# szpajder/dumphfdl

Hardware: AMD Instinct MI355X
Metric: wideband I/Q Msamples/s (cf32 ingest -> decoded HFDL PDUs) at fixed channel count (higher is better)
Workload: dtype f32

## Files before the change

dumphfdl_amd/csrc/demod_core.h:

```cpp
#pragma once
#include <hip/hip_runtime.h>
#include "demod_logic.h"
#include "demod_lds.h"

namespace hfdl {

constexpr int DM_WAVES = 4, DM_THREADS = 64 * DM_WAVES;

__device__ __forceinline__ float dpp_row_shr1(float old, float src)
{
	return __int_as_float(__builtin_amdgcn_update_dpp(__float_as_int(old), __float_as_int(src), 0x111, 0xf, 0xf, false));
}
__device__ __forceinline__ float dpp_row_shl1(float old, float src)
{
	return __int_as_float(__builtin_amdgcn_update_dpp(__float_as_int(old), __float_as_int(src), 0x101, 0xf, 0xf, false));
}
__device__ __forceinline__ float dpp_row_shl2(float old, float src)
{
	return __int_as_float(__builtin_amdgcn_update_dpp(__float_as_int(old), __float_as_int(src), 0x102, 0xf, 0xf, false));
}
__device__ __forceinline__ float dpp_row_ror1(float src)
{
	return __int_as_float(__builtin_amdgcn_update_dpp(0, __float_as_int(src), 0x121, 0xf, 0xf, false));
}
// ... 95 lines not shown

__device__ __forceinline__ cf input_sample(const DemodInput &in, int g)
{
	int b = 0, start = 0;
#pragma unroll
	for (int u = 0; u < DM_MAX_BLOCKS - 1; u++) {
		const int e = in.ends[u];
		if (g >= e) { b = u + 1; start = e; }
	}
	return in.chan[(size_t)b * in.blk_stride + (size_t)(g - start)];
}

template <bool TAPS>
__device__ __forceinline__ void resample_outputs(uint32_t rs_phase, const DemodConst &T, const BlockIo &io, const cf *ring, int k0, int k1, int lane)
{
	const int k = k0 + lane;
	if (k < k1) {
		const uint64_t t = (uint64_t)rs_phase + (uint64_t)k * T.rs_step;
		const int i = (int)(t >> 24);
		const float *h = T.rs_h + ((t & 0xFFFFFFu) >> 16) * D_RS_TAPS;
		float ar = 0, ai = 0;
		for (int j = 0; j < D_RS_TAPS; j++) {
			const cf x = ring[(i - j) & DM_IN_MASK];
			ar += h[j] * x.x;
			ai += h[j] * x.y;
		}
		cf v; v.x = ar; v.y = ai;
		io.rs[k & DM_MASK] = v;
		if (TAPS) io.tap_resampled[k] = v;
	}
}


struct SymsyncRegs {
	float rate, del, tau, bf, q, qhat, v1;
	int b, decim, j;
	int valid_from;
};

__device__ __forceinline__ void symsync_load(SymsyncRegs &r, const ChanScalars &s, const ChanArrays &a, const BlockIo &io, int lane)
{
	if (lane < SS_HIST) {
		cf v; v.x = 0.f; v.y = 0.f;
		if (lane < D_SS_TAPS) v = a.ss_dmf[lane == 0 ? 0 : D_SS_TAPS - lane];
		io.mf[-1 - lane] = v;
	}
	r.rate = s.ss_rate; r.del = s.ss_del; r.tau = s.ss_tau; r.bf = s.ss_bf; r.q = s.ss_q; r.qhat = s.ss_qhat; r.v1 = s.ss_v1;
	r.b = s.ss_b; r.decim = (int)s.ss_decim; r.j = 0;
	r.valid_from = s.ss_head;
}

__device__ __forceinline__ void symsync_restart(SymsyncRegs &r, const DemodShared &sh, int k0)
{
	r.rate = 1.5f; r.del = 1.5f; r.tau = 0.f; r.bf = 0.f; r.q = 0.f; r.qhat = 0.f; r.v1 = 0.f;
	r.b = 0; r.decim = 0;
	r.j = k0 > 0 ? (int)sh.cum[(k0 - 1) & DM_MASK] : 0;
	r.valid_from = k0;
}

__device__ __forceinline__ void symsync_store(const SymsyncRegs &r, ChanScalars &s, ChanArrays &a, const BlockIo &io, int n_out, int lane)
{
	if (lane < D_SS_TAPS) a.ss_dmf[lane == 0 ? 0 : D_SS_TAPS - lane] = io.mf[((n_out - 1) & DM_MASK) - lane];
	if (lane == 0) {
		s.ss_rate = r.rate; s.ss_del = r.del; s.ss_tau = r.tau; s.ss_bf = r.bf; s.ss_q = r.q; s.ss_qhat = r.qhat; s.ss_v1 = r.v1;
		s.ss_b = r.b; s.ss_decim = (uint32_t)r.decim;
		const int vf = r.valid_from - n_out;
		s.ss_head = vf < -64 ? -64 : vf;
	}
}

template <bool MASKED>
__device__ __forceinline__ void symsync_chunk(SymsyncRegs &r, const DemodConst &T, const BlockIo &io, const DemodShared &sh, int k0, int k1, int lane)
{
	const int row = lane >> 4, t = lane & 15;
	const float *base = (const float *)(io.mf - (k0 & ~DM_MASK) - t) + (row & 1);
	int bi = r.b < 0 ? 0 : (r.b >= D_SS_NPFB ? D_SS_NPFB - 1 : r.b);
	float2 h = sh.sstab[bi * 64 + lane];
	float w_lo = base[2 * k0], w_hi = base[2 * (k0 - 16)];
	const bool out_lane = lane == 15 || lane == 31;
	float *const out_base = out_lane ? (float *)sh.outq + (lane == 31 ? 1 : 0) : sh.sink + lane;
	const int out_stride = out_lane ? 2 : 0;
	int cum_v = 0;
	for (int k = k0; k < k1; k++) {
		const float n_lo = base[2 * (k + 1)], n_hi = base[2 * (k + 1 - 16)];
		if (r.b < D_SS_NPFB) {
			float wl = w_lo, wh = w_hi;
			if (MASKED && k - (D_SS_TAPS - 1) < r.valid_from && row < 2) {
				if (k - t < r.valid_from) wl = 0.f;
				if (k - t - 16 < r.valid_from) wh = 0.f;
			}
			int produced = 0;
			do {
				const float p = row_scan_sum(h.x * wl + h.y * wh);
				if (__builtin_expect(r.j < sh.outq_cap, 1)) out_base[out_stride * (r.j & (OUTQ_RING - 1))] = div3(p);
				r.j++;
				if (r.decim == 2) {
					r.decim = 0;
					const float mx = lane_value(p, 15), my = lane_value(p, 31);
					const float dx = lane_value(p, 47), dy = lane_value(p, 63);
					float q = mx * dx + my * dy;
					q = q > 1.0f ? 1.0f : (q < -1.0f ? -1.0f : q);
					r.q = q;
					const float v0 = q - T.lf_a1 * r.v1;
					r.qhat = T.lf_b0 * v0;
					r.v1 = v0;
					r.rate += T.ss_rate_adj * r.qhat;
					r.del = r.rate + r.qhat;
				}
				r.decim++;
				r.tau += r.del;
				r.bf = r.tau * (float)D_SS_NPFB;
				r.b = (int)roundf(r.bf);
				produced++;
				if (r.b < D_SS_NPFB) h = sh.sstab[(r.b < 0 ? 0 : r.b) * 64 + lane];
			} while (r.b < D_SS_NPFB && produced < 4);
		}
		r.tau -= 1.0f;
		r.bf -= (float)D_SS_NPFB;
		r.b -= D_SS_NPFB;
		bi = r.b < 0 ? 0 : (r.b >= D_SS_NPFB ? D_SS_NPFB - 1 : r.b);
		h = sh.sstab[bi * 64 + lane];
		cum_v = (lane == k - k0) ? (r.j < 65535 ? r.j : 65535) : cum_v;
		w_lo = n_lo; w_hi = n_hi;
	}
	if (lane < k1 - k0) sh.cum[(k0 + lane) & DM_MASK] = (uint16_t)cum_v;
}


struct CarrierRegs {
	float eu, ev, ex2, ewx, ewy;
	float px, py;
#ifdef HFDL_DM_PROBE
	unsigned long long pa = 0, pb = 0, pc = 0;
#endif
};

struct LaneSlicer {
	float px, py;
	int lane;
	__device__ __forceinline__ uint32_t operator()(int arity, cf x, float *phase_error) const
	{
		uint32_t sym;
		cf xh;
		if (arity == 1) {
			sym = (x.x > 0) ? 0 : 1;
			xh.x = sym ? -1.0f : 1.0f; xh.y = 0.0f;
		} else {
			const int M = 1 << arity, base = M - 2;
			const bool mine = lane >= base && lane < base + M;
			const float d = mine ? x.x * px + x.y * py : -1.0f;
			const float best = lane_value(row_scan_max(d), 15);
			const unsigned long long hit = __builtin_amdgcn_fcmpf(d, best, 1 );
			int win = hit ? (int)__builtin_ctzll(hit) : base;
			const uint32_t lin = (uint32_t)(win - base);
			sym = lin ^ (lin >> 1);
			xh.x = lane_value(px, win); xh.y = lane_value(py, win);
		}
		if (phase_error) *phase_error = x.y * xh.x - x.x * xh.y;
		return sym;
	}
};

__device__ __forceinline__ void carrier_load(CarrierRegs &c, const ChanScalars &s, const ChanArrays &a, const DemodConst &T, int lane)
{
	c.px = lane < 16 ? T.psk_pts[2 * lane] : 0.f;
	c.py = lane < 16 ? T.psk_pts[2 * lane + 1] : 0.f;
	const int t = (lane & 15) - 1;
	const bool act = t >= 0 && lane < 32, row1 = (lane >> 4) & 1;
	int j = s.eq_head + t; if (j >= D_EQ) j -= D_EQ;
	const cf e = act ? a.eq_buf[j] : cf{0.f, 0.f};
	c.eu = row1 ? e.y : e.x;
	c.ev = row1 ? -e.x : e.y;
	c.ex2 = act ? a.eq_x2[j] : 0.f;
	const cf w = act ? a.eq_w[t] : cf{0.f, 0.f};
	c.ewx = w.x; c.ewy = w.y;
}

__device__ __forceinline__ void carrier_store(const CarrierRegs &c, ChanArrays &a, int lane)
{
	if (lane >= 1 && lane <= D_EQ) {
		cf e; e.x = c.eu; e.y = c.ev;
		a.eq_buf[lane - 1] = e; a.eq_x2[lane - 1] = c.ex2;
		cf w; w.x = c.ewx; w.y = c.ewy;
		a.eq_w[lane - 1] = w;
	}
}

template <bool TAPS>
__device__ __forceinline__ int carrier_chunk(CarrierRegs &c, ChanScalars &s, ChanArrays &a, const DemodConst &T, const BlockIo &io, const DemodShared &sh,
		int k0, int &k1, int &nsym, int lane)
{
	const int t = (lane & 15) - 1;
	const bool row1 = (lane >> 4) & 1, act = t >= 0 && lane < 32;
	int n = k1 - k0;
	const float lv_l = (lane < n) ? io.lvl[(k0 + lane) & DM_MASK] : 0.f;
	const int cum_l = (lane < n) ? (int)sh.cum[(k0 + lane) & DM_MASK] : 0x7fffffff;
	const int jbase = k0 > 0 ? (int)sh.cum[(k0 - 1) & DM_MASK] : 0;
	const cf oq_l = (jbase + lane < sh.outq_cap) ? sh.outq[(jbase + lane) & (OUTQ_RING - 1)] : cf{0.f, 0.f};
	{
#ifndef HFDL_DM_OUT_LANES
#define HFDL_DM_OUT_LANES 64
#endif
		const unsigned long long over = __ballot(lane < n && cum_l - jbase > HFDL_DM_OUT_LANES);
		if (__builtin_expect(over != 0, 0)) { n = (int)__builtin_ctzll(over); k1 = k0 + n; }
	}
	int jstop = __builtin_amdgcn_readlane(cum_l, n - 1);
	if (jstop > sh.outq_cap) jstop = sh.outq_cap;
	const uint64_t cnt0 = s.sample_cnt;
	int kdone = 0;
	int reset_at = -1;
	int staged = 0, stage_at = 0;
	auto flush_stage = [&]() {
		if (lane < staged) io.data[stage_at + lane] = sh.stage[lane];
		staged = 0;
	};
	auto catch_up = [&](int upto) {
		if (s.fr_state == FR_A1) {
			const uint32_t d = (uint32_t)(upto + 1 - kdone), c0 = s.nf_clk;
			uint32_t first = (NF_CLK_MASK - c0) & NF_CLK_MASK;
			if (first == 0) first = NF_CLK_MASK + 1;
			s.nf_clk = (uint32_t)__builtin_amdgcn_readfirstlane((int)(c0 + d));
			if (first <= d) {
				const float level = lane_value(lv_l, kdone + (int)first - 1);
				s.noise_floor = NF_KEEP * s.noise_floor + NF_TAKE * fminf(s.noise_floor, level) + NF_BIAS;
			}
		}
		kdone = upto + 1;
	};
	bool runaway = fabsf(s.dphi) > COSTAS_RUNAWAY_DPHI && s.fr_state == FR_A1;
	const int pair_sel = (lane & 1) << 2;
	auto pair_step = [&](int j) {
		const int sel = ((j - jbase) << 2) + pair_sel;
		cf oi;
		oi.x = __int_as_float(__builtin_amdgcn_ds_bpermute(sel, __float_as_int(oq_l.x)));
		oi.y = __int_as_float(__builtin_amdgcn_ds_bpermute(sel, __float_as_int(oq_l.y)));
		float ph1, ph2;
		{
			const float ph = s.phi + s.dphi;
			const float dn = ph - (float)(2.0 * M_PI), up = ph + (float)(2.0 * M_PI);
			ph1 = ph > (float)M_PI ? dn : (ph < -(float)M_PI ? up : ph);
		}
		{
			const float ph = ph1 + s.dphi;
			const float dn = ph - (float)(2.0 * M_PI), up = ph + (float)(2.0 * M_PI);
			ph2 = ph > (float)M_PI ? dn : (ph < -(float)M_PI ? up : ph);
		}
		s.phi = ph2;
#ifdef HFDL_DM_LIBM_TRIG
		float sp, cp;
		sincosf((lane & 1) ? ph2 : ph1, &sp, &cp);
#else
// ... 24 lines not shown
		const float bx = row1 ? -c.ev : c.eu, by = row1 ? c.eu : c.ev;
		const float pr = er * bx - ei * by, pi = er * by + ei * bx;
		c.ewx = c.ewx + EQ_STEP * pr / s.eq_x2sum;
		c.ewy = c.ewy + EQ_STEP * pi / s.eq_x2sum;
	};
	auto in_frame_run = [&](int &j) {
		if (!(s.symsync_out_idx & 1u) && j + 1 < jstop && s.fr_state >= FR_EQ_TRAIN && s.symbols_wanted > 1 && s.s_state == SAMPLER_SYMBOLS) {
			const bool train = s.fr_state == FR_EQ_TRAIN;
			int n_run = (jstop - j) >> 1;
			if (n_run > s.symbols_wanted - 1) n_run = s.symbols_wanted - 1;
			if ((!train || s.eq_full) && (!s.use_data || s.data_n + n_run <= MAX_DATA_SYMBOLS)) {
				if (s.use_data && staged == 0) stage_at = s.data_slot * MAX_DATA_SYMBOLS + s.data_n;
#if defined(HFDL_DM_PROBE) && HFDL_DM_PROBE >= 2
				const unsigned long long tR0 = __builtin_amdgcn_s_memtime();
#endif
				int ki = 0;
				for (int i = 0; i < n_run; i++, j += 2) {
					pair_step(j);
					const cf y = equalise();
					if (train) { train_step(y); s.T_idx++; }
					if (TAPS && lane == 0) io.tap_symbols[nsym] = y;
					nsym++;
					ki = (int)__builtin_ctzll(__ballot(cum_l > j + 1));
					const float level = lane_value(lv_l, ki);
					float perr;
					LaneSlicer{c.px, c.py, lane}(s.cur_arity, y, &perr);
					const float e = 0.5f * (fabsf(perr + COSTAS_ERR_LIMIT) - fabsf(perr - COSTAS_ERR_LIMIT));
					s.err = e;
					s.phi += COSTAS_ALPHA * e;
					s.dphi += COSTAS_BETA * e;
					if (s.use_data) sh.stage[staged++] = y;
					else if (s.training_n < T_LEN) {
						a.training[s.training_n] = y;
						s.training_n++;
					}
					s.signal_level = (s.signal_level * s.frame_symbol_cnt + level) / (s.frame_symbol_cnt + 1.0f);
					s.frame_symbol_cnt += 1.0f;
				}
				if (ki >= kdone) kdone = ki + 1;
				s.eq_count += 2u * (uint32_t)n_run;
				s.symsync_out_idx += 2u * (uint32_t)n_run;
				s.symbol_cnt += (uint64_t)n_run;
				s.symbols_wanted -= n_run;
				if (s.use_data) s.data_n += n_run;
#if defined(HFDL_DM_PROBE) && HFDL_DM_PROBE >= 2
				{
					const unsigned long long dt = HFDL_DM_PROBE == 2 ? __builtin_amdgcn_s_memtime() - tR0 : (unsigned long long)n_run;
					if (train) c.pb += dt; else c.pc += dt;
				}
#endif
			}
		}
	};
	int j = jbase;
	if (s.fr_state != FR_A1) in_frame_run(j);
	while (j < jstop) {
#ifdef HFDL_DM_PROBE
		const unsigned long long tA0 = __builtin_amdgcn_s_memtime();
		const int st0 = s.fr_state;
#endif
		int jo;
		bool on_time;
		if (!(s.symsync_out_idx & 1u) && j + 1 < jstop && !runaway) {
			pair_step(j);
			s.eq_count += 2;
			jo = j + 1; j += 2; s.symsync_out_idx += 2;
			on_time = true;
		} else {
			cf oi;
			oi.x = lane_value(oq_l.x, j - jbase); oi.y = lane_value(oq_l.y, j - jbase);
			{
				const float ph = s.phi + s.dphi;
				const float dn = ph - (float)(2.0 * M_PI), up = ph + (float)(2.0 * M_PI);
				s.phi = ph > (float)M_PI ? dn : (ph < -(float)M_PI ? up : ph);
			}
#ifdef HFDL_DM_LIBM_TRIG
			float sp, cp;
			sincosf(s.phi, &sp, &cp);
#else
			const float rev = s.phi * 0.15915494309189535f;
			const float sp = __builtin_amdgcn_sinf(rev), cp = __builtin_amdgcn_cosf(rev);
#endif
			cf r;
			r.x = oi.x * cp + oi.y * sp;
			r.y = oi.y * cp - oi.x * sp;
			if (__builtin_expect(runaway, 0)) {
				s.dphi = s.phi = 0.f;
				symsync_reset(s, a);
				runaway = false;
			}
			{
				const float x2n = r.x * r.x + r.y * r.y;
				const float x2o = lane_value(c.ex2, 1);
				const float nu = row1 ? r.y : r.x, nv = row1 ? -r.x : r.y;
				c.eu = dpp_row_shl1(nu, c.eu);
				c.ev = dpp_row_shl1(nv, c.ev);
				c.ex2 = dpp_row_shl1(x2n, c.ex2);
				s.eq_x2sum = s.eq_x2sum + x2n - x2o;
				s.eq_count++;
			}
			on_time = (s.symsync_out_idx & 1u) != 0;
			jo = j; j++; s.symsync_out_idx++;
		}
		if (on_time) {
			const cf y = equalise();
			if (s.fr_state == FR_EQ_TRAIN) {
				bool run = true;
				if (!s.eq_full) { if (s.eq_count < (uint32_t)D_EQ) run = false; else s.eq_full = 1; }
				if (run) train_step(y);
				s.T_idx++;
			}
			if (TAPS && lane == 0) io.tap_symbols[nsym] = y;
			nsym++;
			bool plain = false;
			if (s.fr_state == FR_A1) {
				const bool neg = !(y.x > 0);
				const uint32_t bit = (neg ? 1u : 0u) ^ (s.bitmask & 1u);
				const uint64_t nhi = ((s.bits_hi << 1) | (s.bits_lo >> 63)) & 0x7FFFFFFFFFFFFFFFull, nlo = (s.bits_lo << 1) | bit;
				const int m = bits_correlate(nhi, nlo, T.a_hi, T.a_lo);
				if (__builtin_expect(m > T.a1_lo && m < T.a1_hi && s.s_state == SAMPLER_BITS && s.cur_arity == 1 && s.symbols_wanted <= 1
						&& s.symbol_cnt + 1 < (uint64_t)(NO_FRAME_TIMEOUT_FRAMES * SINGLE_SLOT_FRAME_LEN), 1)) {
					const float perr = y.y * (neg ? -1.0f : 1.0f) - y.x * 0.0f;
					const float e = 0.5f * (fabsf(perr + COSTAS_ERR_LIMIT) - fabsf(perr - COSTAS_ERR_LIMIT));
					s.err = e;
					s.phi += COSTAS_ALPHA * e;
					s.dphi += COSTAS_BETA * e;
					s.symbol_cnt++;
					s.bits_hi = nhi; s.bits_lo = nlo;
					runaway = fabsf(s.dphi) > COSTAS_RUNAWAY_DPHI;
					plain = true;
				}
			}
			else if (s.symbols_wanted > 1) {
				const int ki = (int)__builtin_ctzll(__ballot(cum_l > jo));
				if (ki >= kdone) kdone = ki + 1;
				const float level = lane_value(lv_l, ki);
				float perr;
				uint32_t bits = LaneSlicer{c.px, c.py, lane}(s.cur_arity, y, &perr);
				const float e = 0.5f * (fabsf(perr + COSTAS_ERR_LIMIT) - fabsf(perr - COSTAS_ERR_LIMIT));
				s.err = e;
				s.phi += COSTAS_ALPHA * e;
				s.dphi += COSTAS_BETA * e;
				s.symbol_cnt++;
				if (s.s_state == SAMPLER_SYMBOLS) {
					if (s.use_data) {
						if (s.data_n < MAX_DATA_SYMBOLS) {
							if (staged == 0) stage_at = s.data_slot * MAX_DATA_SYMBOLS + s.data_n;
							sh.stage[staged++] = y;
							s.data_n++;
						}
					} else if (s.training_n < T_LEN) {
						a.training[s.training_n] = y;
						s.training_n++;
					}
				} else if (s.s_state == SAMPLER_BITS) {
					bits ^= s.bitmask;
					for (int b = 0; b < s.cur_arity; b++, bits >>= 1) {
						s.bits_hi = ((s.bits_hi << 1) | (s.bits_lo >> 63)) & 0x7FFFFFFFFFFFFFFFull;
						s.bits_lo = (s.bits_lo << 1) | (bits & 1u);
					}
				}
				s.signal_level = (s.signal_level * s.frame_symbol_cnt + level) / (s.frame_symbol_cnt + 1.0f);
				s.frame_symbol_cnt += 1.0f;
				s.symbols_wanted--;
				runaway = false;
				plain = true;
			}
			if (!plain) {
				if (staged) flush_stage();
				const int ki = (int)__builtin_ctzll(__ballot(cum_l > jo));
				if (ki >= kdone) catch_up(ki);
				const float level = lane_value(lv_l, ki);
				s.sample_cnt = cnt0 + (uint64_t)ki;
				on_symbol(s, *sh.S, a, T, io, y, level, LaneSlicer{c.px, c.py, lane});
				runaway = fabsf(s.dphi) > COSTAS_RUNAWAY_DPHI && s.fr_state == FR_A1;
			}
		}
#if defined(HFDL_DM_PROBE) && HFDL_DM_PROBE >= 2
		{
			const unsigned long long dt = HFDL_DM_PROBE == 2 ? __builtin_amdgcn_s_memtime() - tA0 : 1ull;
			if (st0 == FR_A1) c.pa += dt; else if (st0 == FR_EQ_TRAIN) c.pb += dt; else if (st0 == FR_DATA_1 || st0 == FR_DATA_2) c.pc += dt;
		}
#endif
// ... 27 lines not shown

template <bool TAPS>
__device__ inline int demod_block(ChanArrays &a, const DemodConst &T, const BlockIo &io, const DemodShared &sh, const DemodInput &in)
{
	const int tid = (int)threadIdx.x, wave = tid >> 6, lane = tid & 63;
	ChanScalars &S = *sh.S;
	unsigned long long tR0 = __builtin_amdgcn_s_memtime();

	const uint32_t rs_phase = S.rs_phase;
	const int n_in = in.n_in;
	const uint64_t total = (uint64_t)n_in << 24;
	int n_out = 0;
	if ((uint64_t)rs_phase < total) n_out = (int)((total - rs_phase + T.rs_step - 1) / T.rs_step);
	if (n_out > io.cap - 4) n_out = io.cap - 4;
	auto need = [&](int k_end) {
		return k_end >= n_out ? n_in : (int)(((uint64_t)rs_phase + (uint64_t)(k_end - 1) * T.rs_step) >> 24) + 1;
	};
	auto resampler_store = [&]() {
		cf nh;
		if (lane < D_RS_TAPS - 1) nh = in.ring[(n_in - 1 - lane) & DM_IN_MASK];
		__builtin_amdgcn_wave_barrier();
		if (lane < D_RS_TAPS - 1) a.rs_hist[lane] = nh;
		if (lane == 0) {
			S.rs_phase = (uint32_t)((uint64_t)rs_phase + (uint64_t)n_out * T.rs_step - total);
			if (TAPS) io.tap_counts[0] = n_out;
		}
	};

	if (tid < D_RS_TAPS - 1) in.ring[(-1 - tid) & DM_IN_MASK] = a.rs_hist[tid];
	if (wave == 1 && lane < D_MF - 1) io.agc[(-1 - lane) & DM_AGC_MASK] = a.mf_hist[lane];
	const int rs0 = n_out < DM_CHUNK ? n_out : DM_CHUNK;
	int in_loaded = need(rs0 + 2 * DM_CHUNK);
	for (int g = tid; g < in_loaded; g += DM_THREADS) in.ring[g & DM_IN_MASK] = input_sample(in, g);
	if (TAPS && tid == 0) io.tap_counts[1] = 0;
	__syncthreads();
	if (wave == 3) resample_outputs<TAPS>(rs_phase, T, io, in.ring, 0, rs0, lane);
	__syncthreads();
	if (n_out < 1) {
		if (wave == 3) resampler_store();
		return 0;
	}

	unsigned long long tP0 = __builtin_amdgcn_s_memtime();
	unsigned long long busy = 0;
	int nsym = 0;
#ifdef HFDL_DM_PROBE
	unsigned long long cr_probe[3] = { 0, 0, 0 };
#endif
	PipeProgress pp;
	pp.rs_ready = rs0;
	if (wave == 3) {
		for (int step = 0; pp.s3_done < n_out; step++) {
			int *mb = sh.mbox + 8 * (step & 1);
			int to = pp.rs_ready;
			if (to < n_out) {
				to = to + DM_CHUNK < n_out ? to + DM_CHUNK : n_out;
				if (to > pp.s3_done + DM_RS_AHEAD) to = pp.s3_done + DM_RS_AHEAD;
				const int hi = need(to + 2 * DM_CHUNK < n_out ? to + 2 * DM_CHUNK : n_out);
				cf nx[2];
#pragma unroll
				for (int u = 0; u < 2; u++) {
					const int g = in_loaded + 64 * u + lane;
					nx[u] = g < hi ? input_sample(in, g) : cf{0.f, 0.f};
				}
				resample_outputs<TAPS>(rs_phase, T, io, in.ring, pp.rs_ready, to, lane);
#pragma unroll
				for (int u = 0; u < 2; u++) {
					const int g = in_loaded + 64 * u + lane;
					if (g < hi) in.ring[g & DM_IN_MASK] = nx[u];
				}
				for (int g = in_loaded + 128 + lane; g < hi; g += 64) in.ring[g & DM_IN_MASK] = input_sample(in, g);
				if (hi > in_loaded) in_loaded = hi;
			}
			if (lane == 0) mb[4] = to;
			__syncthreads();
			pp.read(mb);
		}
		resampler_store();
	} else if (wave == 0) {
		float agc_g = S.agc_g, agc_y2 = S.agc_y2;
		for (int step = 0; pp.s3_done < n_out; step++) {
			int *mb = sh.mbox + 8 * (step & 1);
			int to = pp.mf_ready + DM_CHUNK < pp.rs_ready ? pp.mf_ready + DM_CHUNK : pp.rs_ready;
			if (to > pp.s3_done + DM_MF_AHEAD) to = pp.s3_done + DM_MF_AHEAD;
			if (to > pp.mf_ready) agc_mf_chunk<TAPS>(agc_g, agc_y2, T, io, pp.mf_ready, to, lane); else to = pp.mf_ready;
			if (lane == 0) mb[0] = to;
			__syncthreads();
			pp.read(mb);
		}
		cf nh;
		if (lane < D_MF - 1) nh = io.agc[(n_out - 1 - lane) & DM_AGC_MASK];
		__builtin_amdgcn_wave_barrier();
		if (lane < D_MF - 1) a.mf_hist[lane] = nh;
		if (lane == 0) { S.agc_g = agc_g; S.agc_y2 = agc_y2; }
	} else if (wave == 1) {
		SymsyncRegs ss;
		symsync_load(ss, S, a, io, lane);
		__builtin_amdgcn_fence(__ATOMIC_RELEASE, "wavefront");
		__builtin_amdgcn_wave_barrier();
		for (int step = 0; pp.s3_done < n_out; step++) {
			int *mb = sh.mbox + 8 * (step & 1);
			const unsigned long long tb = TAPS ? __builtin_amdgcn_s_memtime() : 0ull;
			if (pp.restart) symsync_restart(ss, sh, pp.ss_ready);
			int to = pp.ss_ready + DM_CHUNK < pp.mf_ready ? pp.ss_ready + DM_CHUNK : pp.mf_ready;
			if (to > pp.s3_done + 2 * DM_CHUNK) to = pp.s3_done + 2 * DM_CHUNK;
			if (to < pp.ss_ready) to = pp.ss_ready;
			for (int k0 = pp.ss_ready; k0 < to;) {
				const int k1 = (k0 | DM_MASK) + 1 < to ? (k0 | DM_MASK) + 1 : to;
				if (__builtin_expect(k0 - (D_SS_TAPS - 1) < ss.valid_from, 0)) symsync_chunk<true>(ss, T, io, sh, k0, k1, lane);
				else symsync_chunk<false>(ss, T, io, sh, k0, k1, lane);
				k0 = k1;
			}
			if (lane == 0) mb[1] = to;
			if (TAPS) busy += __builtin_amdgcn_s_memtime() - tb;
			__syncthreads();
			pp.read(mb);
		}
		if (pp.restart) symsync_restart(ss, sh, n_out);
		symsync_store(ss, S, a, io, n_out, lane);
	} else {
		CarrierRegs cr;
		ChanScalars s3 = S;
		s3.ev_flags = 0;
		carrier_load(cr, s3, a, T, lane);
		for (int step = 0; pp.s3_done < n_out; step++) {
			int *mb = sh.mbox + 8 * (step & 1);
			const unsigned long long tb = TAPS ? __builtin_amdgcn_s_memtime() : 0ull;
			int to = pp.s3_done + DM_CHUNK < pp.ss_ready ? pp.s3_done + DM_CHUNK : pp.ss_ready;
			int reset_at = -1;
			if (to > pp.s3_done) reset_at = carrier_chunk<TAPS>(cr, s3, a, T, io, sh, pp.s3_done, to, nsym, lane); else to = pp.s3_done;
			if (lane == 0) { mb[2] = reset_at >= 0 ? reset_at + 1 : to; mb[3] = reset_at >= 0; }
			if (TAPS) busy += __builtin_amdgcn_s_memtime() - tb;
			__syncthreads();
			pp.read(mb);
		}
		carrier_store(cr, a, lane);
#ifdef HFDL_DM_PROBE
		cr_probe[0] = cr.pa; cr_probe[1] = cr.pb; cr_probe[2] = cr.pc;
#endif
		if (lane == 0) {
			S.phi = s3.phi; S.dphi = s3.dphi; S.err = s3.err;
			S.eq_x2sum = s3.eq_x2sum; S.eq_count = s3.eq_count; S.eq_full = s3.eq_full; S.eq_head = 0;
			S.bits_hi = s3.bits_hi; S.bits_lo = s3.bits_lo;
			S.training_n = s3.training_n; S.data_n = s3.data_n; S.use_data = s3.use_data; S.data_slot = s3.data_slot;
			S.symbol_cnt = s3.symbol_cnt; S.sample_cnt = s3.sample_cnt;
			S.s_state = s3.s_state; S.fr_state = s3.fr_state; S.cur_arity = s3.cur_arity;
			S.symbols_wanted = s3.symbols_wanted; S.T_idx = s3.T_idx;
			S.bitmask = s3.bitmask; S.symsync_out_idx = s3.symsync_out_idx; S.nf_clk = s3.nf_clk;
			S.frame_symbol_cnt = s3.frame_symbol_cnt; S.signal_level = s3.signal_level;
			S.noise_floor = s3.noise_floor;
			S.ev_flags = 0;
			if (TAPS) io.tap_counts[1] = nsym;
		}
	}
	unsigned long long tP1 = __builtin_amdgcn_s_memtime();
	if (TAPS) {
		if (tid == 0) { io.tap_level[io.cap - 4] = (float)(tP0 - tR0); io.tap_level[io.cap - 3] = (float)(tP1 - tP0); }
		if (wave == 1 && lane == 0) io.tap_level[io.cap - 2] = (float)busy;
		if (wave == 2 && lane == 0) io.tap_level[io.cap - 1] = (float)busy;
#ifdef HFDL_DM_PROBE
		__syncthreads();
		if (wave == 2 && lane == 0) { io.tap_level[io.cap - 4] = (float)cr_probe[0]; io.tap_level[io.cap - 3] = (float)cr_probe[1]; io.tap_level[io.cap - 2] = (float)cr_probe[2]; }
#endif
	}
	return n_out;
}

}
```

dumphfdl_amd/csrc/demod_logic.h:

```cpp
#pragma once
#include <stdint.h>
#include <math.h>

#define HFDL_FN __device__ inline
#define HFDL_HD __host__ __device__ inline
#ifndef HFDL_ATAN2F
#define HFDL_ATAN2F atan2f
#endif

namespace hfdl {

struct cf { float x, y; };

constexpr int D_RS_NPFB = 256, D_RS_TAPS = 14, D_SS_NPFB = 16, D_SS_TAPS = 18, D_EQ = 15, D_MF = 19;
constexpr int MAX_DATA_SYMBOLS = 168 * 30;

constexpr int PREKEY_LEN = 448, A_LEN = 127, M1_LEN = 127, M2_LEN = 15, T_LEN = 15, DATA_FRAME_LEN = 30, PREAMBLE_T_SEQS = 9;
constexpr int SINGLE_SLOT_FRAME_LEN = PREKEY_LEN + (2 * A_LEN + M1_LEN + M2_LEN + PREAMBLE_T_SEQS * T_LEN) + 72 * (DATA_FRAME_LEN + T_LEN);
constexpr float CORR_THRESHOLD_A1 = 0.36f, CORR_THRESHOLD_A2 = 0.3f, CORR_THRESHOLD_M1 = 0.3f;
constexpr int MAX_SEARCH_RETRIES = 3, NO_FRAME_TIMEOUT_FRAMES = 13;
constexpr int HFDL_SYMBOL_RATE = 1800, HFDL_SPS = 3;
constexpr float COSTAS_ALPHA = 0.1f, COSTAS_BETA = 0.047f * COSTAS_ALPHA * COSTAS_ALPHA;
constexpr float COSTAS_ERR_LIMIT = 1.0f, COSTAS_RUNAWAY_DPHI = 0.25f;
constexpr float AGC_BANDWIDTH = 0.01f, EQ_STEP = 0.1f;
// ... 33 lines not shown
	float frame_symbol_cnt, freq_err_hz, signal_level, noise_floor;
	uint32_t cnt_a2_found, cnt_m1_found, cnt_m1_not_found, cnt_frames;
	uint32_t cnt_a1_found, sum_a1_dev, sum_a2_dev, sum_m1_dev, cum_train_bad, cum_train_total;
	uint32_t ev_flags;
};
enum { EV_SS_RESET = 1, EV_EQ_RESET = 2 };

struct ChanArrays {
	cf rs_hist[D_RS_TAPS - 1];
	cf mf_hist[D_MF - 1];
	cf ss_mf[D_SS_TAPS], ss_dmf[D_SS_TAPS];
	cf eq_w[D_EQ], eq_buf[D_EQ];
	float eq_x2[D_EQ];
	cf training[T_LEN];
};

struct ChanState { ChanScalars s; ChanArrays a; };

struct FrameRec {
	int32_t channel, slot, mode, bitmask_lsb;
	float freq_err_hz, signal_level, noise_floor;
	int32_t train_bad, train_total, pad;
	uint64_t sample_index;
};

struct DemodConst {
	const float *rs_h;
	uint32_t rs_step;
	const float *mf;
	const float *ss_mf, *ss_dmf;
	float lf_b0, lf_a1, ss_rate_adj;
	const float *eq_h0;
	uint64_t a_hi, a_lo;
	const uint64_t *m1_hi, *m1_lo;
	const float *corr_tab;
	const float *psk_pts;
	int32_t a1_lo, a1_hi, a2_lo, a2_hi, pos_min;
};

struct BlockIo {
	cf *rs, *agc, *mf;
	float *lvl;
	int cap;
	cf *data;
	FrameRec *frames;
	int *frame_count;
	int frame_cap;
	cf *tap_resampled, *tap_mf, *tap_symbols;
	float *tap_level;
	int *tap_counts;
	int channel;
};

HFDL_HD void chan_state_init(ChanState &st, const float *eq_h0)
{
	ChanScalars &s = st.s;
	ChanArrays &a = st.a;
	char *p = (char *)&st;
	for (unsigned i = 0; i < sizeof(ChanState); i++) p[i] = 0;
	s.agc_g = 1.0f; s.agc_y2 = 1.0f;
	s.noise_floor = 1.0f;
	s.ss_rate = 1.5f; s.ss_del = 1.5f;
	for (int i = 0; i < D_EQ; i++) { a.eq_w[i].x = eq_h0[i]; a.eq_w[i].y = 0.f; }
	s.fr_state = FR_A1; s.symbols_wanted = 1; s.cur_arity = 1; s.s_state = SAMPLER_BITS;
}


HFDL_FN uint32_t gray_enc(uint32_t b) { return b ^ (b >> 1); }
HFDL_FN uint32_t gray_dec(uint32_t g) { uint32_t b = g; while (g >>= 1) b ^= g; return b; }

HFDL_FN int psk_entry(int arity, uint32_t lin) { return (1 << arity) - 2 + (int)lin; }

struct PskTable {
	const float *p;
	HFDL_FN cf operator()(int i) const { cf y; y.x = p[2 * i]; y.y = p[2 * i + 1]; return y; }
};

template <class Pts>
HFDL_FN uint32_t psk_slice(int arity, cf x, float *phase_error, const Pts &pts)
{
	uint32_t sym;
	cf xh;
	if (arity == 1) {
		sym = (x.x > 0) ? 0 : 1;
		xh.x = sym ? -1.0f : 1.0f; xh.y = 0.0f;
	} else {
		const uint32_t M = 1u << arity;
		const float alpha = (float)M_PI / (float)M;
		float theta = HFDL_ATAN2F(x.y, x.x);
		theta -= (float)M_PI * (1.0f - 1.0f / (float)M);
		if (theta < -(float)M_PI) theta += 2 * (float)M_PI;
		uint32_t s = 0;
		float v = theta;
		for (int k = arity - 1; k >= 0; k--) {
			const float ref = (float)(1u << k) * alpha;
			s <<= 1;
			if (v > 0) { s |= 1; v -= ref; } else { v += ref; }
		}
		sym = gray_enc(s);
		xh = pts(psk_entry(arity, s));
	}
	if (phase_error) *phase_error = x.y * xh.x - x.x * xh.y;
	return sym;
}

HFDL_FN uint8_t soft_clamp(float v)
{
	int s = (int)(v + 127);
	return (uint8_t)(s > 255 ? 255 : (s < 0 ? 0 : s));
}

struct TableSlicer {
	const float *p;
	HFDL_FN uint32_t operator()(int arity, cf x, float *phase_error) const { return psk_slice(arity, x, phase_error, PskTable{p}); }
};
// ... 70 lines not shown
	}
	*hdr_len_out = hdr_len;
	if (len < hdr_len + 2) return 2;
	const uint16_t rx = (uint16_t)(buf[hdr_len] | (buf[hdr_len + 1] << 8));
	return rx == crc16_x25(buf, hdr_len) ? 0 : 1;
}

struct LpduCounts { uint8_t processed, good, bad_fcs, too_short, truncated; };

HFDL_FN int lpdu_list_walk(const uint8_t *lens, const uint8_t *data, const uint8_t *end, uint32_t lpdu_cnt, LpduCounts &c)
{
	int consumed = 0;
	for (uint32_t j = 0; j < lpdu_cnt; j++) {
		const uint32_t lpdu_len = (uint32_t)lens[j] + 1;
		if (data + lpdu_len > end) { c.truncated = 1; return -1; }
		c.processed++;
		if (lpdu_len < 3) c.too_short++;
		else {
			const uint16_t rx = (uint16_t)(data[lpdu_len - 2] | (data[lpdu_len - 1] << 8));
			if (rx == crc16_x25(data, lpdu_len - 2)) c.good++; else c.bad_fcs++;
		}
		data += lpdu_len;
		consumed += (int)lpdu_len;
	}
	return consumed;
}

HFDL_FN LpduCounts lpdu_walk(const uint8_t *buf, uint32_t len, int kind, uint32_t hdr_len)
{
	LpduCounts c;
	c.processed = c.good = c.bad_fcs = c.too_short = c.truncated = 0;
	const uint8_t *end = buf + len;
	const uint8_t *data = buf + hdr_len + 2;
	if (kind == 1) {
		lpdu_list_walk(buf + 6, data, end, (buf[0] >> 2) & 0xFu, c);
	} else if (kind == 2) {
		const uint32_t aircraft_cnt = ((buf[0] & 0x70u) >> 4) + 1;
		const uint8_t *hdr = buf + 2;
		for (uint32_t i = 0; i < aircraft_cnt; i++) {
			hdr++;
			const uint32_t lpdu_cnt = (*hdr++ >> 4) & 0xFu;
			const int used = lpdu_list_walk(hdr, data, end, lpdu_cnt, c);
			if (used < 0) break;
			hdr += lpdu_cnt;
			data += used;
		}
	}
	return c;
}

HFDL_FN void symsync_reset(ChanScalars &s, ChanArrays &a)
{
	for (int i = 0; i < D_SS_TAPS; i++) { a.ss_mf[i].x = 0.f; a.ss_mf[i].y = 0.f; }
	s.ss_rate = 1.5f; s.ss_del = 1.5f;
	s.ss_b = 0; s.ss_bf = 0.f; s.ss_tau = 0.f; s.ss_q = 0.f; s.ss_qhat = 0.f;
	s.ss_decim = 0; s.ss_v1 = 0.f;
	s.ev_flags |= EV_SS_RESET;
}

HFDL_FN void eq_reset(ChanScalars &s, ChanArrays &a, const float *eq_h0)
{
	for (int i = 0; i < D_EQ; i++) {
		a.eq_w[i].x = eq_h0[i]; a.eq_w[i].y = 0.f;
		a.eq_buf[i].x = 0.f; a.eq_buf[i].y = 0.f;
		a.eq_x2[i] = 0.f;
	}
	s.eq_x2sum = 0.f; s.eq_count = 0; s.eq_full = 0; s.eq_head = 0;
	s.ev_flags |= EV_EQ_RESET;
}

HFDL_FN void framer_reset(ChanScalars &s, ChanScalars &c, ChanArrays &a, const float *eq_h0)
{
	s.fr_state = FR_A1;
	s.symbols_wanted = 1;
	c.search_retries = 0;
	s.cur_arity = 1;
	c.train_total = c.train_bad = 0;
	s.T_idx = 0;
	s.use_data = 0;
	eq_reset(s, a, eq_h0);
	s.data_n = 0;
	s.training_n = 0;
	symsync_reset(s, a);
	s.s_state = SAMPLER_BITS;
	s.bitmask = 0;
}

HFDL_FN int bits_correlate(uint64_t hi, uint64_t lo, uint64_t thi, uint64_t tlo)
{
	return 127 - __popcll((hi ^ thi) & 0x7FFFFFFFFFFFFFFFull) - __popcll(lo ^ tlo);
}

HFDL_HD float t_symbol(int idx)
{
	if (idx > T_LEN - 1) idx = T_LEN - 1;
	return ((T_SEQ_BITS >> (T_LEN - 1 - idx)) & 1u) ? -1.0f : 1.0f;
}

template <class Slicer>
HFDL_FN void on_symbol(ChanScalars &s, ChanScalars &c, ChanArrays &a, const DemodConst &T, const BlockIo &io, cf sym, float level, const Slicer &slice)
{
	float perr;
	uint32_t bits = slice(s.cur_arity, sym, &perr);
	{
		const float e = 0.5f * (fabsf(perr + COSTAS_ERR_LIMIT) - fabsf(perr - COSTAS_ERR_LIMIT));
		s.err = e;
		s.phi += COSTAS_ALPHA * e;
// ... 177 lines not shown
```

Baseline: 18940.

## Streamline symsync inner loop and batch A1 search symbols in carrier stage

The symbol-sync loop now uses a pointer-increment window and a single unconditional output step, with the rarely taken extra-output loop moved behind an unlikely branch. roundf becomes add-copysign-truncate, and the divide-by-three moves from the per-output symsync store to the carrier-stage outq load. A new search_run lambda processes consecutive on-time symbol pairs during the A1 preamble search in a tight loop instead of going around the general per-symbol dispatcher. The change also adds probe instrumentation and a profiling script. It risks subtle state-accounting differences (symbol_cnt, eq_count) in the batched search path.

Measured after the change: 19870 (median of 6 runs). +5.0%, better.

```diff
diff --git a/dumphfdl_amd/csrc/demod_core.h b/dumphfdl_amd/csrc/demod_core.h
--- a/dumphfdl_amd/csrc/demod_core.h
+++ b/dumphfdl_amd/csrc/demod_core.h
@@ -171,7 +171,7 @@
 
 __device__ __forceinline__ void symsync_restart(SymsyncRegs &r, const DemodShared &sh, int k0)
 {
-	r.rate = 1.5f; r.del = 1.5f; r.tau = 0.f; r.bf = 0.f; r.q = 0.f; r.qhat = 0.f; r.v1 = 0.f;
+	r.rate = HFDL_DM_SS_RATE0; r.del = HFDL_DM_SS_RATE0; r.tau = 0.f; r.bf = 0.f; r.q = 0.f; r.qhat = 0.f; r.v1 = 0.f;
 	r.b = 0; r.decim = 0;
 	r.j = k0 > 0 ? (int)sh.cum[(k0 - 1) & DM_MASK] : 0;
 	r.valid_from = k0;
@@ -192,53 +192,59 @@
 __device__ __forceinline__ void symsync_chunk(SymsyncRegs &r, const DemodConst &T, const BlockIo &io, const DemodShared &sh, int k0, int k1, int lane)
 {
 	const int row = lane >> 4, t = lane & 15;
-	const float *base = (const float *)(io.mf - (k0 & ~DM_MASK) - t) + (row & 1);
-	int bi = r.b < 0 ? 0 : (r.b >= D_SS_NPFB ? D_SS_NPFB - 1 : r.b);
-	float2 h = sh.sstab[bi * 64 + lane];
-	float w_lo = base[2 * k0], w_hi = base[2 * (k0 - 16)];
+	const float *wp = (const float *)(io.mf - (k0 & ~DM_MASK) - t - 16) + (row & 1) + 2 * k0;
+	const float2 *const hp = sh.sstab + lane;
+	float2 h = hp[(r.b < 0 ? 0 : (r.b >= D_SS_NPFB ? D_SS_NPFB - 1 : r.b)) * 64];
+	float w_lo = wp[32], w_hi = wp[0];
 	const bool out_lane = lane == 15 || lane == 31;
-	float *const out_base = out_lane ? (float *)sh.outq + (lane == 31 ? 1 : 0) : sh.sink + lane;
-	const int out_stride = out_lane ? 2 : 0;
+	char *const out_base = out_lane ? (char *)((float *)sh.outq + (lane == 31 ? 1 : 0)) : (char *)(sh.sink + lane);
+	const uint32_t out_stride = out_lane ? (uint32_t)sizeof(cf) : 0u;
 	int cum_v = 0;
-	for (int k = k0; k < k1; k++) {
-		const float n_lo = base[2 * (k + 1)], n_hi = base[2 * (k + 1 - 16)];
+	auto output_step = [&](float wl, float wh) {
+		const float p = row_scan_sum(h.x * wl + h.y * wh);
+		if (__builtin_expect(r.j < sh.outq_cap, 1)) *(float *)(out_base + out_stride * (uint32_t)(r.j & (OUTQ_RING - 1))) = p;
+		r.j++;
+		const bool filter = r.decim == 2;
+		r.decim = filter ? 1 : r.decim + 1;
+		if (filter) {
+			const float mx = lane_value(p, 15), my = lane_value(p, 31);
+			const float dx = lane_value(p, 47), dy = lane_value(p, 63);
+			float q = mx * dx + my * dy;
+			q = q > 1.0f ? 1.0f : (q < -1.0f ? -1.0f : q);
+			r.q = q;
+			const float v0 = q - T.lf_a1 * r.v1;
+			r.qhat = T.lf_b0 * v0;
+			r.v1 = v0;
+			r.rate += T.ss_rate_adj * r.qhat;
+			r.del = r.rate + r.qhat;
+		}
+		r.tau += r.del;
+		r.bf = r.tau * (float)D_SS_NPFB;
+		r.b = (int)(r.bf + __builtin_copysignf(0x1.fffffep-2f, r.bf));
+	};
+	for (int k = k0; k < k1; k++, wp += 2) {
+		const float n_lo = wp[34], n_hi = wp[2];
 		if (r.b < D_SS_NPFB) {
 			float wl = w_lo, wh = w_hi;
 			if (MASKED && k - (D_SS_TAPS - 1) < r.valid_from && row < 2) {
 				if (k - t < r.valid_from) wl = 0.f;
 				if (k - t - 16 < r.valid_from) wh = 0.f;
 			}
-			int produced = 0;
-			do {
-				const float p = row_scan_sum(h.x * wl + h.y * wh);
-				if (__builtin_expect(r.j < sh.outq_cap, 1)) out_base[out_stride * (r.j & (OUTQ_RING - 1))] = div3(p);
-				r.j++;
-				if (r.decim == 2) {
-					r.decim = 0;
-					const float mx = lane_value(p, 15), my = lane_value(p, 31);
-					const float dx = lane_value(p, 47), dy = lane_value(p, 63);
-					float q = mx * dx + my * dy;
-					q = q > 1.0f ? 1.0f : (q < -1.0f ? -1.0f : q);
-					r.q = q;
-					const float v0 = q - T.lf_a1 * r.v1;
-					r.qhat = T.lf_b0 * v0;
-					r.v1 = v0;
-					r.rate += T.ss_rate_adj * r.qhat;
-					r.del = r.rate + r.qhat;
-				}
-				r.decim++;
-				r.tau += r.del;
-				r.bf = r.tau * (float)D_SS_NPFB;
-				r.b = (int)roundf(r.bf);
-				produced++;
-				if (r.b < D_SS_NPFB) h = sh.sstab[(r.b < 0 ? 0 : r.b) * 64 + lane];
-			} while (r.b < D_SS_NPFB && produced < 4);
+			output_step(wl, wh);
+			if (__builtin_expect(r.b < D_SS_NPFB, 0)) {
+				int produced = 1;
+				do {
+					h = hp[(r.b < 0 ? 0 : r.b) * 64];
+					output_step(wl, wh);
+					produced++;
+				} while (r.b < D_SS_NPFB && produced < 4);
+			}
 		}
 		r.tau -= 1.0f;
 		r.bf -= (float)D_SS_NPFB;
 		r.b -= D_SS_NPFB;
-		bi = r.b < 0 ? 0 : (r.b >= D_SS_NPFB ? D_SS_NPFB - 1 : r.b);
-		h = sh.sstab[bi * 64 + lane];
+		const int lo = r.b > 0 ? r.b : 0;
+		h = hp[(lo < D_SS_NPFB - 1 ? lo : D_SS_NPFB - 1) * 64];
 		cum_v = (lane == k - k0) ? (r.j < 65535 ? r.j : 65535) : cum_v;
 		w_lo = n_lo; w_hi = n_hi;
 	}
@@ -315,7 +321,8 @@
 	const float lv_l = (lane < n) ? io.lvl[(k0 + lane) & DM_MASK] : 0.f;
 	const int cum_l = (lane < n) ? (int)sh.cum[(k0 + lane) & DM_MASK] : 0x7fffffff;
 	const int jbase = k0 > 0 ? (int)sh.cum[(k0 - 1) & DM_MASK] : 0;
-	const cf oq_l = (jbase + lane < sh.outq_cap) ? sh.outq[(jbase + lane) & (OUTQ_RING - 1)] : cf{0.f, 0.f};
+	cf oq_l = (jbase + lane < sh.outq_cap) ? sh.outq[(jbase + lane) & (OUTQ_RING - 1)] : cf{0.f, 0.f};
+	oq_l.x = div3(oq_l.x); oq_l.y = div3(oq_l.y);
 	{
 #ifndef HFDL_DM_OUT_LANES
 #define HFDL_DM_OUT_LANES 64
@@ -446,6 +453,40 @@
 			}
 		}
 	};
+	struct SearchRunEnd { bool finished; int jo; cf y; };
+	auto search_run = [&](int &j, int jo, cf y) {
+		bool finished = true;
+		const uint64_t room = (uint64_t)(NO_FRAME_TIMEOUT_FRAMES * SINGLE_SLOT_FRAME_LEN) - 1u - s.symbol_cnt;
+		const int n_left = room > 64u ? 64 : (int)room;
+		int n_run = 0;
+		while (j + 1 < jstop && !runaway) {
+			pair_step(j);
+			jo = j + 1; j += 2;
+			y = equalise();
+			if (TAPS && lane == 0) io.tap_symbols[nsym] = y;
+			nsym++;
+			const bool neg = !(y.x > 0);
+			const uint32_t bit = (neg ? 1u : 0u) ^ (s.bitmask & 1u);
+			const uint64_t nhi = ((s.bits_hi << 1) | (s.bits_lo >> 63)) & 0x7FFFFFFFFFFFFFFFull, nlo = (s.bits_lo << 1) | bit;
+			const int m = bits_correlate(nhi, nlo, T.a_hi, T.a_lo);
+			n_run++;
+			if (__builtin_expect(!(m > T.a1_lo && m < T.a1_hi && n_run <= n_left), 0)) { finished = false; break; }
+			const float perr = y.y * (neg ? -1.0f : 1.0f) - y.x * 0.0f;
+			const float e = 0.5f * (fabsf(perr + COSTAS_ERR_LIMIT) - fabsf(perr - COSTAS_ERR_LIMIT));
+			s.err = e;
+			s.phi += COSTAS_ALPHA * e;
+			s.dphi += COSTAS_BETA * e;
+			s.bits_hi = nhi; s.bits_lo = nlo;
+			runaway = fabsf(s.dphi) > COSTAS_RUNAWAY_DPHI;
+		}
+		s.eq_count += 2u * (uint32_t)n_run;
+		s.symsync_out_idx += 2u * (uint32_t)n_run;
+		s.symbol_cnt += (uint64_t)(finished ? n_run : n_run - 1);
+#if defined(HFDL_DM_PROBE) && HFDL_DM_PROBE == 3
+		c.pa += (unsigned long long)n_run;
+#endif
+		return SearchRunEnd{finished, jo, y};
+	};
 	int j = jbase;
 	if (s.fr_state != FR_A1) in_frame_run(j);
 	while (j < jstop) {
@@ -497,7 +538,7 @@
 			jo = j; j++; s.symsync_out_idx++;
 		}
 		if (on_time) {
-			const cf y = equalise();
+			cf y = equalise();
 			if (s.fr_state == FR_EQ_TRAIN) {
 				bool run = true;
 				if (!s.eq_full) { if (s.eq_count < (uint32_t)D_EQ) run = false; else s.eq_full = 1; }
@@ -522,7 +563,8 @@
 					s.symbol_cnt++;
 					s.bits_hi = nhi; s.bits_lo = nlo;
 					runaway = fabsf(s.dphi) > COSTAS_RUNAWAY_DPHI;
-					plain = true;
+					const SearchRunEnd end = search_run(j, jo, y);
+					plain = end.finished; jo = end.jo; y = end.y;
 				}
 			}
 			else if (s.symbols_wanted > 1) {
@@ -656,6 +698,9 @@
 	if (wave == 3) {
 		for (int step = 0; pp.s3_done < n_out; step++) {
 			int *mb = sh.mbox + 8 * (step & 1);
+#if defined(HFDL_DM_PROBE) && HFDL_DM_PROBE == 5
+			const unsigned long long tb = __builtin_amdgcn_s_memtime();
+#endif
 			int to = pp.rs_ready;
 			if (to < n_out) {
 				to = to + DM_CHUNK < n_out ? to + DM_CHUNK : n_out;
@@ -677,6 +722,9 @@
 				if (hi > in_loaded) in_loaded = hi;
 			}
 			if (lane == 0) mb[4] = to;
+#if defined(HFDL_DM_PROBE) && HFDL_DM_PROBE == 5
+			busy += __builtin_amdgcn_s_memtime() - tb;
+#endif
 			__syncthreads();
 			pp.read(mb);
 		}
@@ -685,10 +733,18 @@
 		float agc_g = S.agc_g, agc_y2 = S.agc_y2;
 		for (int step = 0; pp.s3_done < n_out; step++) {
 			int *mb = sh.mbox + 8 * (step & 1);
+#if defined(HFDL_DM_PROBE) && (HFDL_DM_PROBE == 4 || HFDL_DM_PROBE == 6)
+			const unsigned long long tb = __builtin_amdgcn_s_memtime();
+#endif
 			int to = pp.mf_ready + DM_CHUNK < pp.rs_ready ? pp.mf_ready + DM_CHUNK : pp.rs_ready;
 			if (to > pp.s3_done + DM_MF_AHEAD) to = pp.s3_done + DM_MF_AHEAD;
 			if (to > pp.mf_ready) agc_mf_chunk<TAPS>(agc_g, agc_y2, T, io, pp.mf_ready, to, lane); else to = pp.mf_ready;
 			if (lane == 0) mb[0] = to;
+#if defined(HFDL_DM_PROBE) && HFDL_DM_PROBE == 4
+			busy += __builtin_amdgcn_s_memtime() - tb;
+#elif defined(HFDL_DM_PROBE) && HFDL_DM_PROBE == 6
+			if (lane == 0) mb[5] = (int)(__builtin_amdgcn_s_memtime() - tb);
+#endif
 			__syncthreads();
 			pp.read(mb);
 		}
@@ -717,6 +773,9 @@
 			}
 			if (lane == 0) mb[1] = to;
 			if (TAPS) busy += __builtin_amdgcn_s_memtime() - tb;
+#if defined(HFDL_DM_PROBE) && HFDL_DM_PROBE == 6
+			if (TAPS && lane == 0) mb[6] = (int)(__builtin_amdgcn_s_memtime() - tb);
+#endif
 			__syncthreads();
 			pp.read(mb);
 		}
@@ -735,11 +794,20 @@
 			if (to > pp.s3_done) reset_at = carrier_chunk<TAPS>(cr, s3, a, T, io, sh, pp.s3_done, to, nsym, lane); else to = pp.s3_done;
 			if (lane == 0) { mb[2] = reset_at >= 0 ? reset_at + 1 : to; mb[3] = reset_at >= 0; }
 			if (TAPS) busy += __builtin_amdgcn_s_memtime() - tb;
+#if defined(HFDL_DM_PROBE) && HFDL_DM_PROBE == 6
+			if (TAPS && lane == 0) mb[7] = (int)(__builtin_amdgcn_s_memtime() - tb);
+#endif
 			__syncthreads();
 			pp.read(mb);
+#if defined(HFDL_DM_PROBE) && HFDL_DM_PROBE == 6
+			{
+				const int m01 = mb[5] > mb[6] ? mb[5] : mb[6];
+				cr_probe[0] += (unsigned long long)(m01 > mb[7] ? m01 : mb[7]);
+			}
+#endif
 		}
 		carrier_store(cr, a, lane);
-#ifdef HFDL_DM_PROBE
+#if defined(HFDL_DM_PROBE) && HFDL_DM_PROBE != 6
 		cr_probe[0] = cr.pa; cr_probe[1] = cr.pb; cr_probe[2] = cr.pc;
 #endif
 		if (lane == 0) {
@@ -764,7 +832,13 @@
 		if (wave == 2 && lane == 0) io.tap_level[io.cap - 1] = (float)busy;
 #ifdef HFDL_DM_PROBE
 		__syncthreads();
+#if HFDL_DM_PROBE == 2 || HFDL_DM_PROBE == 3
 		if (wave == 2 && lane == 0) { io.tap_level[io.cap - 4] = (float)cr_probe[0]; io.tap_level[io.cap - 3] = (float)cr_probe[1]; io.tap_level[io.cap - 2] = (float)cr_probe[2]; }
+#elif HFDL_DM_PROBE == 4 || HFDL_DM_PROBE == 5
+		if (wave == (HFDL_DM_PROBE == 4 ? 0 : 3) && lane == 0) io.tap_level[io.cap - 4] = (float)busy;
+#elif HFDL_DM_PROBE == 6
+		if (wave == 2 && lane == 0) io.tap_level[io.cap - 4] = (float)cr_probe[0];
+#endif
 #endif
 	}
 	return n_out;
diff --git a/dumphfdl_amd/csrc/demod_logic.h b/dumphfdl_amd/csrc/demod_logic.h
--- a/dumphfdl_amd/csrc/demod_logic.h
+++ b/dumphfdl_amd/csrc/demod_logic.h
@@ -109,6 +109,10 @@
 	int channel;
 };
 
+#ifndef HFDL_DM_SS_RATE0
+#define HFDL_DM_SS_RATE0 1.5f
+#endif
+
 HFDL_HD void chan_state_init(ChanState &st, const float *eq_h0)
 {
 	ChanScalars &s = st.s;
@@ -117,7 +121,7 @@
 	for (unsigned i = 0; i < sizeof(ChanState); i++) p[i] = 0;
 	s.agc_g = 1.0f; s.agc_y2 = 1.0f;
 	s.noise_floor = 1.0f;
-	s.ss_rate = 1.5f; s.ss_del = 1.5f;
+	s.ss_rate = HFDL_DM_SS_RATE0; s.ss_del = HFDL_DM_SS_RATE0;
 	for (int i = 0; i < D_EQ; i++) { a.eq_w[i].x = eq_h0[i]; a.eq_w[i].y = 0.f; }
 	s.fr_state = FR_A1; s.symbols_wanted = 1; s.cur_arity = 1; s.s_state = SAMPLER_BITS;
 }
@@ -294,7 +298,7 @@
 HFDL_FN void symsync_reset(ChanScalars &s, ChanArrays &a)
 {
 	for (int i = 0; i < D_SS_TAPS; i++) { a.ss_mf[i].x = 0.f; a.ss_mf[i].y = 0.f; }
-	s.ss_rate = 1.5f; s.ss_del = 1.5f;
+	s.ss_rate = HFDL_DM_SS_RATE0; s.ss_del = HFDL_DM_SS_RATE0;
 	s.ss_b = 0; s.ss_bf = 0.f; s.ss_tau = 0.f; s.ss_q = 0.f; s.ss_qhat = 0.f;
 	s.ss_decim = 0; s.ss_v1 = 0.f;
 	s.ev_flags |= EV_SS_RESET;
diff --git a/profiles/wave_cycles.py b/profiles/wave_cycles.py
--- /dev/null
+++ b/profiles/wave_cycles.py
@@ -0,0 +1,85 @@
+#!/usr/bin/env python3
+import json
+import os
+import subprocess
+import sys
+
+sys.path.insert(0, os.path.dirname(os.path.dirname(os.path.abspath(__file__))))
+import numpy as np
+
+FS, CF, FREQ = 250000, 10_000_000, 10_021_000
+FR_A1, FR_EQ_TRAIN = 1, 5
+LAUNCH = 512
+COLS = ("P", "W0", "W1", "W2", "W3", "S")
+
+
+def child():
+    import hfdl_synth as synth
+    import dumphfdl_amd as hf
+    from dumphfdl_amd import frontend as F
+    from oracle import pyoracle
+    rows = []
+    for mode in (1, 2, 3):
+        rng = np.random.default_rng(300 + mode)
+        b = dict(freq=FREQ, mode=mode, octets=synth.make_pdu(rng, mode), t0=1.1, amp=0.1, cfo=(-1) ** mode * (3.0 + mode))
+        n = int((b["t0"] + synth.burst_symbols_len(mode) / 1800.0 + 0.3) * FS)
+        x = synth.synth_wideband(FS, CF, n, [b], noise_sigma=0.004, seed=70 + mode)
+        ora = pyoracle.Frontend(FS, CF, [FREQ])
+        size, parts = ora.ddc.input_size, []
+        for i in range(len(x) // size):
+            ora.push_block(x[i * size:(i + 1) * size])
+            parts.append(np.array(ora.channel_view(0)["chan_out"], np.complex64))
+        ora.close()
+        chan = np.concatenate(parts)
+        fe = hf.Frontend(FS, CF, [FREQ])
+        step = int(round(float(1 << 24) / float(fe.geometry.resamp_rate)))
+        n_in = (LAUNCH * step) >> 24
+        before, in_t = fe.channel_stats(0), 0
+        for at in range(0, len(chan) - n_in + 1, n_in):
+            fe.push_baseband([chan[at:at + n_in]])
+            cyc = np.array(fe.read_tap(F.TAP_PHASE_CYCLES, 0), np.float64)
+            n_out = len(fe.read_tap(F.TAP_AGC_LEVEL, 0))
+            after = fe.channel_stats(0)
+            s0, s1 = before["framer_state"], after["framer_state"]
+            if s0 == s1 == FR_A1 and before["frames"] == after["frames"] and before["a2_found"] == after["a2_found"]:
+                kind, in_t = "search", 0
+            elif s0 >= FR_EQ_TRAIN and s1 >= FR_EQ_TRAIN and before["frames"] == after["frames"]:
+                in_t += 1
+                kind = "mode %d preamble T" % mode if in_t <= 2 else "mode %d data" % mode
+            else:
+                kind = "mixed"
+            rows.append((kind, (cyc / n_out).tolist()))
+            before = after
+        fe.poll_pdus()
+        fe.close()
+    print(json.dumps(rows))
+
+
+def main(arms):
+    table = {}
+    names = []
+    for arm in arms:
+        name, libs = arm.split("=")
+        names.append(name)
+        for slot0, lib in zip(("W0", "W3", "S"), libs.split(",")):
+            r = subprocess.run([sys.executable, os.path.abspath(__file__), "--child"], env=dict(os.environ, HFDL_GPU_LIB=os.path.abspath(lib)),
+                               capture_output=True, text=True, timeout=300)
+            if r.returncode != 0:
+                sys.exit("%s: exit %d\n%s" % (lib, r.returncode, r.stderr[-2000:]))
+            for kind, c in json.loads(r.stdout.strip().splitlines()[-1]):
+                t = table.setdefault(kind, {}).setdefault(name, {k: [] for k in COLS})
+                t[slot0].append(c[0]); t["P"].append(c[1]); t["W1"].append(c[2]); t["W2"].append(c[3])
+    print("cycles per 5400-sps sample, min - max over the launches of a class (P, W1, W2: over both builds of the arm)")
+    print("| state (launches) | arm | P | W0 | W1 | W2 | W3 | S |\n|---|---|---|---|---|---|---|---|")
+    for kind in sorted(table):
+        for name in names:
+            t = table[kind].get(name)
+            if t:
+                print("| %s (%d) | %s | %s |" % (kind, len(t["W0"]), name, " | ".join("%.0f - %.0f" % (min(t[k]), max(t[k])) if t[k] else "" for k in COLS)))
+
+
+if __name__ == "__main__":
+    if len(sys.argv) > 1 and sys.argv[1] == "--child":
+        child()
+    else:
+        main(sys.argv[1:])
```
